# DavidHan008/SLAM-1

Hardware: AMD Instinct MI355X
Metric: frames/sec tracking+local-BA @1280x720 (higher is better)
Workload: dtype u8+f32+f64

## Files before the change

### include/slam355.h

```cpp
#ifndef SLAM355_H
#define SLAM355_H

#include <stddef.h>
#include <stdint.h>

#ifdef __cplusplus
extern "C" {
#endif

#define SLAM355_ABI_VERSION 1

#define SLAM_OK 0
#define SLAM_ERR_ARG (-1)
#define SLAM_ERR_HIP (-2)
#define SLAM_ERR_WORKSPACE (-3)
#define SLAM_ERR_COMM (-4)

int slam_abi_version(void);
const char* slam_last_error(void);
int slam_device_count(void);

int slam_hamming_knn2(const uint8_t* d_q, const int32_t* d_nq, int q_cap,
                      const uint8_t* d_t, const int32_t* d_nt, int t_cap,
                      int batch, int32_t* d_idx2, int32_t* d_dist2,
// ... 19 lines not shown

int slam_fundamental_lmeds(const double* d_m1, const double* d_m2, const int32_t* d_count,
                           int cap, int batch, uint64_t seed, int item0, int n_hyp,
                           uint8_t* d_mask, double* d_F, int32_t* d_ninliers, void* stream);
int slam_fundamental_lmeds_ws(const double* d_m1, const double* d_m2, const int32_t* d_count,
                              int cap, int batch, uint64_t seed, int item0, int n_hyp,
                              uint8_t* d_mask, double* d_F, int32_t* d_ninliers, double* d_ws,
                              long long ws_len, void* stream);
long long slam_fundamental_workspace_len(int batch, int n_hyp);

int slam_filter_pairs(const int32_t* d_pairs, const int32_t* d_count, const uint8_t* d_mask,
                      int cap, int batch, int32_t* d_out, int32_t* d_out_count, void* stream);

int slam_triangulate(const double* d_ptl, const double* d_ptr, const int32_t* d_count, int cap,
                     int batch, const double* d_Pl, const double* d_Pr, int proj_stride,
                     double* d_X, void* stream);

int slam_pnp_ransac(const double* d_Q, const double* d_q, const int32_t* d_count, int cap,
                    int batch, const double* d_K, uint64_t seed, int item0, int n_hyp,
                    double reproj_thresh, int hyp_iters, int refine_iters, double* d_rvec,
                    double* d_tvec, int32_t* d_ninliers, uint8_t* d_mask, double* d_ws,
                    long long ws_len, void* stream);
long long slam_pnp_workspace_len(int batch, int n_hyp);

int slam_pose_chain(const double* d_rvec, const double* d_tvec, const int32_t* d_ninliers,
                    int batch, double* d_state, double* d_poses, void* stream);

int slam_vo_estimate_pose(const double* d_q1, const double* d_q2, const double* d_Q1,
                          const double* d_Q2, const int32_t* d_count, int cap, int batch,
                          const double* d_P, uint64_t seed, int item0, int max_iter,
                          int lm_iters, int early_stop, double* d_pose, int32_t* d_best,
                          int32_t* d_ntried, double* d_err, void* d_ws, size_t ws_bytes,
                          void* stream);
int slam_vo_pose_workspace_bytes(int batch, int max_iter, size_t* bytes);

int slam_vo_residuals(const double* d_dof, const double* d_q1, const double* d_q2,
                      const double* d_Q1, const double* d_Q2, const int32_t* d_count, int cap,
                      int batch, const double* d_P, double* d_res, void* stream);

int slam_rel_to_abs(const double* d_rel, const int32_t* d_count, int cap, int batch,
                    const double* d_poses, double* d_abs, void* stream);

int slam_map_workspace_bytes(int max_queries, int map_cap, size_t* bytes);
int slam_map_associate(double* d_map, int32_t* d_M, int map_cap, int M_bound,
                       const double* d_abs, const double* d_rel, const double* d_pts2d,
                       const int32_t* d_n, int N, double threshold, int frame_index,
// ... 218 lines not shown
```

### slam-1_amd/csrc/epnp.hpp

```cpp
#pragma once

#include <hip/hip_runtime.h>
#include <cmath>

namespace slam_epnp {

constexpr int EPNP_MAXN = 8;
constexpr int kEpnpWs = 4 * EPNP_MAXN + 48 + 60;

template <int n>
__device__ __forceinline__ void ep_jacobi(double* A, double* V) {
  #pragma unroll
  for (int i = 0; i < n; ++i)
    #pragma unroll
    for (int j = 0; j < n; ++j) V[i * n + j] = i == j ? 1.0 : 0.0;
  #pragma unroll 1
  for (int sweep = 0; sweep < 40; ++sweep) {
    double off = 0.0, dia = 0.0;
    #pragma unroll
    for (int i = 0; i < n; ++i) {
      dia += A[i * n + i] * A[i * n + i];
      #pragma unroll
      for (int j = i + 1; j < n; ++j) off += A[i * n + j] * A[i * n + j];
    }
    if (!(off > 1e-30 * dia)) break;
    constexpr int kUnroll = n <= 4 ? 4 : 1;
// ... 218 lines not shown
  } else if (R[0] > R[4] && R[0] > R[8]) {
    const double s = 2.0 * sqrt(1.0 + R[0] - R[4] - R[8]);
    q0 = (R[7] - R[5]) / s; q1 = 0.25 * s; q2 = (R[1] + R[3]) / s; q3 = (R[2] + R[6]) / s;
  } else if (R[4] > R[8]) {
    const double s = 2.0 * sqrt(1.0 + R[4] - R[0] - R[8]);
    q0 = (R[2] - R[6]) / s; q1 = (R[1] + R[3]) / s; q2 = 0.25 * s; q3 = (R[5] + R[7]) / s;
  } else {
    const double s = 2.0 * sqrt(1.0 + R[8] - R[0] - R[4]);
    q0 = (R[3] - R[1]) / s; q1 = (R[2] + R[6]) / s; q2 = (R[5] + R[7]) / s; q3 = 0.25 * s;
  }
  if (q0 < 0.0) {
    q0 = -q0; q1 = -q1; q2 = -q2; q3 = -q3;
  }
  const double vn = sqrt(q1 * q1 + q2 * q2 + q3 * q3);
  const double th = 2.0 * atan2(vn, q0);
  const double k = vn > 0.0 ? th / vn : 2.0;
  r[0] = q1 * k; r[1] = q2 * k; r[2] = q3 * k;
}

constexpr int kJld = 13;
struct EpGroup {
  double A[144], V[144];
  double alph[4 * EPNP_MAXN];
  double v[4][12];
  double L[60], rho[6];
  double cw[4][3];
  double res[3][8];
  double offdia[2];
  double B[2][12 * kJld];
  double cs[12];
  double part[24];
  double pad[27];
  int flag;
};
static_assert(sizeof(EpGroup) % 256 == 128, "EpGroup stride must be 128 mod 256 bytes");

template <int n>
__device__ __forceinline__ int ep_bary(const double* pw, EpGroup& G) {
  double cw[4][3] = {{0, 0, 0}};
  for (int i = 0; i < n; ++i)
    for (int d = 0; d < 3; ++d) cw[0][d] += pw[3 * i + d];
  for (int d = 0; d < 3; ++d) cw[0][d] /= n;
  double A3[9] = {0, 0, 0, 0, 0, 0, 0, 0, 0}, V3[9];
  for (int i = 0; i < n; ++i)
    for (int a = 0; a < 3; ++a)
      for (int b = 0; b < 3; ++b) A3[3 * a + b] += (pw[3 * i + a] - cw[0][a]) * (pw[3 * i + b] - cw[0][b]);
  ep_jacobi<3>(A3, V3);
  int ord[3] = {0, 1, 2};
  for (int i = 0; i < 3; ++i)
    for (int j = i + 1; j < 3; ++j)
      if (A3[4 * ord[j]] > A3[4 * ord[i]]) {
        const int tmp = ord[i]; ord[i] = ord[j]; ord[j] = tmp;
      }
  for (int k = 0; k < 3; ++k) {
    const double sc = sqrt(fmax(A3[4 * ord[k]], 0.0) / n);
    for (int d = 0; d < 3; ++d) cw[k + 1][d] = cw[0][d] + sc * V3[3 * d + ord[k]];
  }
  for (int k = 0; k < 4; ++k)
// ... 186 lines not shown
    ep_jacobi_round<0>(G, k, kr, act, cur, vr);
    ep_jacobi_round<1>(G, k, kr, act, cur ^ 1, vr);
    ep_jacobi_round<2>(G, k, kr, act, cur, vr);
    ep_jacobi_round<3>(G, k, kr, act, cur ^ 1, vr);
    ep_jacobi_round<4>(G, k, kr, act, cur, vr);
    ep_jacobi_round<5>(G, k, kr, act, cur ^ 1, vr);
    ep_jacobi_round<6>(G, k, kr, act, cur, vr);
    ep_jacobi_round<7>(G, k, kr, act, cur ^ 1, vr);
    ep_jacobi_round<8>(G, k, kr, act, cur, vr);
    ep_jacobi_round<9>(G, k, kr, act, cur ^ 1, vr);
    ep_jacobi_round<10>(G, k, kr, act, cur, vr);
    cur ^= 1;
  }
  if (own) {
#pragma unroll
    for (int j = 0; j < n; ++j) {
      G.A[k * n + j] = G.B[cur][k * ld + j];
      G.V[k * n + j] = vr[j];
    }
  }
  __syncthreads();
}

__device__ __forceinline__ void ep_lrho(EpGroup& G) {
  int o12[12];
  for (int i = 0; i < 12; ++i) o12[i] = i;
  for (int i = 0; i < 4; ++i)
    for (int j = i + 1; j < 12; ++j)
      if (G.A[13 * o12[j]] < G.A[13 * o12[i]]) {
        const int tmp = o12[i]; o12[i] = o12[j]; o12[j] = tmp;
      }
  for (int k = 0; k < 4; ++k)
    for (int r = 0; r < 12; ++r) G.v[k][r] = G.V[12 * r + o12[k]];
  const int pa[6] = {0, 0, 0, 1, 1, 2}, pb[6] = {1, 2, 3, 2, 3, 3};
  for (int j = 0; j < 6; ++j) {
    double dv[4][3];
    for (int k = 0; k < 4; ++k)
      for (int d = 0; d < 3; ++d) dv[k][d] = G.v[k][3 * pa[j] + d] - G.v[k][3 * pb[j] + d];
#define EP_DOT(a, b) (dv[a][0] * dv[b][0] + dv[a][1] * dv[b][1] + dv[a][2] * dv[b][2])
    G.L[10 * j + 0] = EP_DOT(0, 0);
    G.L[10 * j + 1] = 2.0 * EP_DOT(0, 1);
    G.L[10 * j + 2] = EP_DOT(1, 1);
    G.L[10 * j + 3] = 2.0 * EP_DOT(0, 2);
    G.L[10 * j + 4] = 2.0 * EP_DOT(1, 2);
    G.L[10 * j + 5] = EP_DOT(2, 2);
    G.L[10 * j + 6] = 2.0 * EP_DOT(0, 3);
    G.L[10 * j + 7] = 2.0 * EP_DOT(1, 3);
    G.L[10 * j + 8] = 2.0 * EP_DOT(2, 3);
    G.L[10 * j + 9] = EP_DOT(3, 3);
#undef EP_DOT
    double s = 0.0;
    for (int d = 0; d < 3; ++d) {
      const double e = G.cw[pa[j]][d] - G.cw[pb[j]][d];
      s += e * e;
    }
    G.rho[j] = s;
  }
}

template <int n>
__device__ __forceinline__ void ep_approx(int approx, const double* pw, const double* uv, double fx,
                                          double fy, double cx, double cy, EpGroup& G) {
  double* res = G.res[approx];
  res[7] = 0.0;
  const int k = approx == 0 ? 4 : approx == 1 ? 3 : 5;
  double As[30], xb[5], rho[6];
#pragma unroll
  for (int j = 0; j < 6; ++j) rho[j] = G.rho[j];
#pragma unroll
  for (int j = 0; j < 6; ++j)
#pragma unroll
    for (int c = 0; c < 5; ++c) {
      const int col = c < 2 ? c : approx == 0 ? (c == 2 ? 3 : 6) : c;
      As[j * 5 + c] = c < k ? G.L[10 * j + col] : 0.0;
    }
  if (!ep_lsq6_live(As, rho, k, xb)) return;
  double be[4] = {0, 0, 0, 0};
  if (approx == 0) {
    if (xb[0] < 0.0) {
      be[0] = sqrt(-xb[0]);
      be[1] = -xb[1] / be[0]; be[2] = -xb[2] / be[0]; be[3] = -xb[3] / be[0];
    } else {
      be[0] = sqrt(xb[0]);
      be[1] = xb[1] / be[0]; be[2] = xb[2] / be[0]; be[3] = xb[3] / be[0];
    }
// ... 21 lines not shown
      Ag[4 * j + 3] = l[6] * be[0] + l[7] * be[1] + l[8] * be[2] + 2.0 * l[9] * be[3];
      bg[j] = rho[j] - (l[0] * be[0] * be[0] + l[1] * be[0] * be[1] + l[2] * be[1] * be[1] +
                        l[3] * be[0] * be[2] + l[4] * be[1] * be[2] + l[5] * be[2] * be[2] +
                        l[6] * be[0] * be[3] + l[7] * be[1] * be[3] + l[8] * be[2] * be[3] +
                        l[9] * be[3] * be[3]);
    }
    if (!ep_lsq6<4>(Ag, bg, dx)) break;
    for (int c = 0; c < 4; ++c) be[c] += dx[c];
  }
  double ccs[4][3];
  for (int j = 0; j < 4; ++j)
    for (int d = 0; d < 3; ++d)
      ccs[j][d] = be[0] * G.v[0][3 * j + d] + be[1] * G.v[1][3 * j + d] + be[2] * G.v[2][3 * j + d] +
                  be[3] * G.v[3][3 * j + d];
  double R[9], t[3];
  res[0] = ep_pose<n>(ccs, G.alph, pw, uv, fx, fy, cx, cy, R, t);
  double r[3];
  ep_rvec(R, r);
  res[1] = r[0]; res[2] = r[1]; res[3] = r[2];
  res[4] = t[0]; res[5] = t[1]; res[6] = t[2];
  res[7] = 1.0;
}

__device__ __forceinline__ int ep_choose(const EpGroup& G, double p[6]) {
  double best_err = INFINITY;
  int ok = 0;
  for (int a = 0; a < 3; ++a) {
    if (G.res[a][7] == 0.0) continue;
    if (G.res[a][0] < best_err) {
      best_err = G.res[a][0];
      for (int i = 0; i < 6; ++i) p[i] = G.res[a][1 + i];
      ok = 1;
    }
  }
  for (int i = 0; i < 6; ++i) ok &= isfinite(p[i]) ? 1 : 0;
  return ok;
}

}
```

### slam-1_amd/csrc/geometry.hip

```cpp
#include "common.hpp"
#include "epnp.hpp"
#include "dlt.hpp"

#include <climits>

#include <cmath>

namespace {

constexpr int kBS = 256;

__global__ __launch_bounds__(kBS) void k_gather(const float* __restrict__ kpq, int kq_cap,
                                                const float* __restrict__ kpt, int kt_cap,
                                                const uint8_t* __restrict__ dq_in,
                                                const uint8_t* __restrict__ dt_in,
                                                const int2* __restrict__ pairs,
                                                const int32_t* __restrict__ count, int p_cap,
                                                double* __restrict__ ptq, double* __restrict__ ptt,
                                                uint8_t* __restrict__ dq, uint8_t* __restrict__ dt) {
  const int b = blockIdx.y;
  const int n = min(max(count[b], 0), p_cap);
  const int k = blockIdx.x * kBS + threadIdx.x;
  if (k >= n) return;
  const size_t o = (size_t)b * p_cap + k;
// ... 269 lines not shown
__device__ __forceinline__ void allsum_halve(double (&v)[32], int lane) {
  constexpr int half = OFF / 2;
  const bool hi = (lane & OFF) != 0;
#pragma unroll
  for (int k = 0; k < half; ++k) {
    const double send = hi ? v[k] : v[k + half];
    const double keep = hi ? v[k + half] : v[k];
    v[k] = keep + __shfl_xor(send, OFF, 64);
  }
}
__device__ __forceinline__ void wave_allsum32(double (&v)[32]) {
  const int lane = threadIdx.x & 63;
  allsum_halve<32>(v, lane);
  allsum_halve<16>(v, lane);
  allsum_halve<8>(v, lane);
  allsum_halve<4>(v, lane);
  allsum_halve<2>(v, lane);
  const double tot = v[0] + __shfl_xor(v[0], 1, 64);
#pragma unroll
  for (int j = 0; j < 32; ++j) v[j] = readlane_d(tot, 2 * j);
}

constexpr int kHypGroups = 4;
#ifdef SLAM_PNPH_TRACE
__device__ unsigned long long g_pnph[8];
#define PNPH_T(i) do { if (threadIdx.x == 0 && blockIdx.x == 3 && blockIdx.y == 5) g_pnph[i] = __builtin_amdgcn_s_memtime(); } while (0)
#else
#define PNPH_T(i) (void)0
#endif
__device__ void pnp_sample(uint64_t seed, int item, int h, int L, const double* Q, const double* q,
                           double* pw, double* uv, int* sidx) {
  uint64_t s = seed ^ ((uint64_t)item * 0xD1B54A32D192ED03ull) ^
               ((uint64_t)h * 0x8CB92BA72F3D8DD7ull);
  int idx[kMinSample];
  for (int kk = 0; kk < kMinSample; ++kk) {
    int v;
    bool dup;
    do {
      v = (int)((splitmix64(s) >> 32) % (uint64_t)L);
      dup = false;
      for (int j = 0; j < kk; ++j) dup |= idx[j] == v;
    } while (dup);
    idx[kk] = v;
    sidx[kk] = v;
    for (int d = 0; d < 3; ++d) pw[3 * kk + d] = Q[3 * v + d];
    for (int d = 0; d < 2; ++d) uv[2 * kk + d] = q[2 * v + d];
  }
}

__global__ __launch_bounds__(64) void k_pnp_hyp(const double* __restrict__ Qall,
                                                const double* __restrict__ qall,
                                                const int32_t* __restrict__ count, int cap,
                                                const double* __restrict__ Kp, uint64_t seed,
                                                int item0, int n_hyp, double* __restrict__ ws) {
#ifdef SLAM_PNP_PRIO
  __builtin_amdgcn_s_setprio(SLAM_PNP_PRIO);
#endif
  __shared__ slam_epnp::EpGroup grp[kHypGroups];
  __shared__ double spw[kHypGroups][3 * kMinSample], suv[kHypGroups][2 * kMinSample];
  __shared__ int sidx[kHypGroups][kMinSample];
  const int b = blockIdx.x, t = threadIdx.x;
  const int g = t >> 4, k = t & 15;
  const int h = blockIdx.y * kHypGroups + g;
  const int L = min(max(count[b], 0), cap);
  if (L < kMinSample) return;
  const bool live = h < n_hyp;
  const double* Q = Qall + (size_t)b * cap * 3;
  const double* q = qall + (size_t)b * cap * 2;
  const Cam K{Kp[0], Kp[4], Kp[2], Kp[5]};
  slam_epnp::EpGroup& G = grp[g];
  PNPH_T(0);
  if (k == 0 && live) {
    pnp_sample(seed, item0 + b, h, L, Q, q, spw[g], suv[g], sidx[g]);
    G.flag = slam_epnp::ep_bary<kMinSample>(spw[g], G);
  }
  __syncthreads();
  PNPH_T(1);
  bool ok = live && G.flag != 0;
  if (ok && k < 12) slam_epnp::ep_mtm_row<kMinSample>(k, suv[g], K.fx, K.fy, K.cx, K.cy, G);
  __syncthreads();
  PNPH_T(2);
  slam_epnp::ep_jacobi12_group(G, k, ok);
  PNPH_T(3);
#ifdef SLAM_PNPH_TRACE
  if (threadIdx.x == 0 && blockIdx.x == 3 && blockIdx.y == 5) g_pnph[7] = (unsigned long long)G.offdia[1];
#endif
  if (ok && k == 0) slam_epnp::ep_lrho(G);
  __syncthreads();
  PNPH_T(4);
  if (ok && k < 3) slam_epnp::ep_approx<kMinSample>(k, spw[g], suv[g], K.fx, K.fy, K.cx, K.cy, G);
  __syncthreads();
  PNPH_T(5);
  if (k == 0 && live) {
    double p[6] = {0, 0, 0, 0, 0, 0};
    if (!(ok && slam_epnp::ep_choose(G, p)))
      for (int i = 0; i < 6; ++i) p[i] = 0.0;
    double* o = ws + ((size_t)b * n_hyp + h) * 6;
    for (int i = 0; i < 6; ++i) o[i] = p[i];
  }
  PNPH_T(6);
}

__global__ __launch_bounds__(64) void k_pnp_hyp_lm(const double* __restrict__ Qall,
                                                   const double* __restrict__ qall,
                                                   const int32_t* __restrict__ count, int cap,
                                                   const double* __restrict__ Kp, uint64_t seed,
                                                   int item0, int n_hyp, int hyp_iters,
                                                   double* __restrict__ ws) {
#ifdef SLAM_PNP_PRIO
  __builtin_amdgcn_s_setprio(SLAM_PNP_PRIO);
#endif
  __shared__ double spw[kHypGroups][3 * kMinSample], suv[kHypGroups][2 * kMinSample];
  __shared__ int sidx[kHypGroups][kMinSample];
  __shared__ double lmt[kHypGroups * kLmGroup], lms[kHypGroups][28 + kMinSample];
  __shared__ double p0[kHypGroups][6];
  const int b = blockIdx.x, t = threadIdx.x;
  const int g = t >> 4, k = t & 15;
  const int h = blockIdx.y * kHypGroups + g;
  const int L = min(max(count[b], 0), cap);
  if (L < kMinSample) return;
  const bool live = h < n_hyp;
  const double* Q = Qall + (size_t)b * cap * 3;
  const double* q = qall + (size_t)b * cap * 2;
// ... 610 lines not shown
      d_Q1, d_q2, d_q1);
  SLAM_LAUNCHED("k_gather_temporal");
  return SLAM_OK;
}

extern "C" int slam_triangulate(const double* d_ptl, const double* d_ptr, const int32_t* d_count,
                                int cap, int batch, const double* d_Pl, const double* d_Pr,
                                int proj_stride, double* d_X, void* stream) {
  SLAM_REQUIRE(batch >= 0 && cap >= 0, "slam_triangulate: bad shape");
  SLAM_REQUIRE(proj_stride == 0 || proj_stride == 12, "slam_triangulate: proj_stride 0 or 12");
  if (batch == 0 || cap == 0) return SLAM_OK;
  SLAM_REQUIRE(d_ptl && d_ptr && d_count && d_Pl && d_Pr && d_X, "slam_triangulate: null pointer");
  dim3 grid((cap + kBS - 1) / kBS, batch);
  k_triangulate<<<grid, kBS, 0, slam::as_stream(stream)>>>(d_ptl, d_ptr, d_count, cap, d_Pl, d_Pr,
                                                           proj_stride, d_X);
  SLAM_LAUNCHED("k_triangulate");
  return SLAM_OK;
}

extern "C" long long slam_pnp_workspace_len(int batch, int n_hyp) {
  return (long long)batch * n_hyp * 6;
}

extern "C" int slam_pnp_ransac(const double* d_Q, const double* d_q, const int32_t* d_count,
                               int cap, int batch, const double* d_K, uint64_t seed, int item0,
                               int n_hyp, double reproj_thresh, int hyp_iters, int refine_iters,
                               double* d_rvec, double* d_tvec, int32_t* d_ninliers,
                               uint8_t* d_mask, double* d_ws, long long ws_len, void* stream) {
  SLAM_REQUIRE(batch >= 0 && cap >= 0, "slam_pnp_ransac: bad shape");
  SLAM_REQUIRE(n_hyp >= 1 && n_hyp <= kMaxHyp, "slam_pnp_ransac: n_hyp in [1, %d]", kMaxHyp);
  SLAM_REQUIRE(hyp_iters >= 0 && refine_iters >= 0 && reproj_thresh > 0,
               "slam_pnp_ransac: bad iteration/threshold arguments");
  if (batch == 0) return SLAM_OK;
  SLAM_REQUIRE(d_Q && d_q && d_count && d_K && d_rvec && d_tvec && d_ninliers && d_mask && d_ws,
               "slam_pnp_ransac: null pointer");
  if (ws_len < slam_pnp_workspace_len(batch, n_hyp)) {
    slam::set_error("slam_pnp_ransac: workspace %lld < %lld doubles", ws_len,
                    slam_pnp_workspace_len(batch, n_hyp));
    return SLAM_ERR_WORKSPACE;
  }
  hipStream_t s = slam::as_stream(stream);
  const dim3 hgrid(batch, (n_hyp + kHypGroups - 1) / kHypGroups);
  k_pnp_hyp<<<hgrid, 64, 0, s>>>(d_Q, d_q, d_count, cap, d_K, seed, item0, n_hyp, d_ws);
  SLAM_LAUNCHED("k_pnp_hyp");
  k_pnp_hyp_lm<<<hgrid, 64, 0, s>>>(d_Q, d_q, d_count, cap, d_K, seed, item0, n_hyp, hyp_iters,
                                    d_ws);
  SLAM_LAUNCHED("k_pnp_hyp_lm");
  k_pnp<<<batch, kPnPWG, 0, s>>>(d_Q, d_q, d_count, cap, d_K, seed, item0, n_hyp, reproj_thresh,
                                 hyp_iters, refine_iters, d_rvec, d_tvec, d_ninliers, d_mask,
                                 d_ws);
  SLAM_LAUNCHED("k_pnp");
  return SLAM_OK;
}

extern "C" int slam_vo_pose_workspace_bytes(int batch, int max_iter, size_t* bytes) {
  SLAM_REQUIRE(batch >= 0 && max_iter >= 1 && bytes, "slam_vo_pose_workspace_bytes: bad args");
  *bytes = (size_t)batch * max_iter * 7 * sizeof(double) + 256;
  return SLAM_OK;
}

extern "C" int slam_vo_estimate_pose(const double* d_q1, const double* d_q2, const double* d_Q1,
                                     const double* d_Q2, const int32_t* d_count, int cap,
                                     int batch, const double* d_P, uint64_t seed, int item0,
                                     int max_iter, int lm_iters, int early_stop, double* d_pose,
                                     int32_t* d_best, int32_t* d_ntried, double* d_err,
                                     void* d_ws, size_t ws_bytes, void* stream) {
  SLAM_REQUIRE(batch >= 0 && cap >= 0, "slam_vo_estimate_pose: bad shape");
  SLAM_REQUIRE(max_iter >= 1 && max_iter <= kVoWG, "slam_vo_estimate_pose: max_iter in [1, %d]",
               kVoWG);
  SLAM_REQUIRE(lm_iters >= 0 && early_stop >= 1, "slam_vo_estimate_pose: bad lm_iters/early_stop");
  if (batch == 0) return SLAM_OK;
  SLAM_REQUIRE(d_q1 && d_q2 && d_Q1 && d_Q2 && d_count && d_P && d_pose && d_best && d_ntried &&
                   d_err,
               "slam_vo_estimate_pose: null pointer");
  SLAM_REQUIRE(d_ws != nullptr, "slam_vo_estimate_pose: null workspace");
// ... 29 lines not shown
               "slam_vo_residuals: null pointer");
  dim3 grid((4 * cap + kBS - 1) / kBS, batch);
  k_vo_residuals<<<grid, kBS, 0, slam::as_stream(stream)>>>(d_dof, d_q1, d_q2, d_Q1, d_Q2,
                                                           d_count, cap, d_P, d_res);
  SLAM_LAUNCHED("k_vo_residuals");
  return SLAM_OK;
}

extern "C" int slam_pose_chain(const double* d_rvec, const double* d_tvec,
                               const int32_t* d_ninliers, int batch, double* d_state,
                               double* d_poses, void* stream) {
  SLAM_REQUIRE(batch >= 0, "slam_pose_chain: batch < 0");
  if (batch == 0) return SLAM_OK;
  SLAM_REQUIRE(d_rvec && d_tvec && d_ninliers && d_state && d_poses, "slam_pose_chain: null pointer");
  k_pose_chain<<<1, 64, 0, slam::as_stream(stream)>>>(d_rvec, d_tvec, d_ninliers, batch, d_state,
                                                     d_poses);
  SLAM_LAUNCHED("k_pose_chain");
  return SLAM_OK;
}

#ifdef SLAM_PNPH_TRACE
extern "C" int slam_pnph_trace(unsigned long long* out) {
  SLAM_HIP(hipDeviceSynchronize());
  SLAM_HIP(hipMemcpyFromSymbol(out, HIP_SYMBOL(g_pnph), 8 * sizeof(unsigned long long)));
  return SLAM_OK;
}
#endif
```

### slam-1_amd/slam355/_lib.py

```python
from __future__ import annotations

import ctypes
import os

_HERE = os.path.dirname(os.path.abspath(__file__))
LIB_PATH = os.environ.get("SLAM355_LIB") or os.path.join(_HERE, "libslam355.so")

c_int = ctypes.c_int
c_double = ctypes.c_double
c_size_t = ctypes.c_size_t
c_p = ctypes.c_void_p
c_uint64 = ctypes.c_uint64
c_longlong = ctypes.c_longlong

c_i32 = ctypes.c_int32


class BAProblemStruct(ctypes.Structure):
    _fields_ = [
        ("n_cams", c_i32), ("n_pts", c_i32), ("n_obs", c_i32), ("n_grps", c_i32),
        ("n_blocks", c_i32), ("n_cslots", c_i32), ("n_bslots", c_i32), ("lin_mode", c_i32),
        ("n_sgrps", c_i32), ("tl_mode", c_i32),
        ("cams", c_p * 2), ("pts", c_p * 2), ("camrec", c_p * 2),
        ("obs_cam", c_p), ("obs_pt", c_p), ("obs_q", c_p), ("pt_ptr", c_p), ("grp_ptr", c_p),
# ... 24 lines not shown
        ("n_cslots", c_i32), ("n_bslots", c_i32), ("n_blocks", c_i32), ("chunks_per_wg", c_i32),
        ("off", ctypes.c_longlong * len(PLAN_TABLES)), ("len", ctypes.c_longlong * len(PLAN_TABLES)),
        ("total", ctypes.c_longlong),
    ]

SIGNATURES = {
    "slam_abi_version": [],
    "slam_last_error": [],
    "slam_device_count": [],
    "slam_hamming_knn2": [c_p, c_p, c_int, c_p, c_p, c_int, c_int, c_p, c_p, c_p, c_p],
    "slam_compact_matches": [c_p, c_p, c_p, c_int, c_int, c_p, c_double, c_p, c_p, c_p],
    "slam_orb_workspace_bytes": [c_int, c_int, c_int, c_int, c_int, c_int, c_int,
                                 ctypes.POINTER(c_size_t)],
    "slam_orb_tiles": [c_p, c_int, c_int, c_int, c_int, c_int, c_int, c_int, c_int, c_p,
                       c_size_t, c_p, c_p, c_p, c_p, c_int, c_p],
    "slam_gather_matches": [c_p, c_int, c_p, c_int, c_p, c_p, c_p, c_p, c_int, c_int, c_p, c_p,
                            c_p, c_p, c_p],
    "slam_gather_temporal": [c_p, c_p, c_int, c_p, c_int, c_p, c_p, c_int, c_int, c_p, c_p, c_p,
                             c_p],
    "slam_triangulate": [c_p, c_p, c_p, c_int, c_int, c_p, c_p, c_int, c_p, c_p],
    "slam_pnp_ransac": [c_p, c_p, c_p, c_int, c_int, c_p, c_uint64, c_int, c_int, c_double, c_int,
                        c_int, c_p, c_p, c_p, c_p, c_p, c_longlong, c_p],
    "slam_pnp_workspace_len": [c_int, c_int],
    "slam_pose_chain": [c_p, c_p, c_p, c_int, c_p, c_p, c_p],
    "slam_vo_estimate_pose": [c_p, c_p, c_p, c_p, c_p, c_int, c_int, c_p, c_uint64, c_int, c_int,
                              c_int, c_int, c_p, c_p, c_p, c_p, c_p, c_size_t, c_p],
    "slam_vo_pose_workspace_bytes": [c_int, c_int, ctypes.POINTER(c_size_t)],
    "slam_vo_residuals": [c_p, c_p, c_p, c_p, c_p, c_p, c_int, c_int, c_p, c_p, c_p],
    "slam_map_workspace_bytes": [c_int, c_int, ctypes.POINTER(c_size_t)],
    "slam_rel_to_abs": [c_p, c_p, c_int, c_int, c_p, c_p, c_p],
    "slam_map_windows": [c_p, c_p, c_int, c_int, c_int, c_p, c_p, c_p, c_p, c_int, c_double, c_p,
                         c_p, c_size_t, c_p],
    "slam_map_associate": [c_p, c_p, c_int, c_int, c_p, c_p, c_p, c_p, c_int, c_double, c_int,
                           c_p, c_p, c_size_t, c_p],
    "slam_fundamental_lmeds": [c_p, c_p, c_p, c_int, c_int, c_uint64, c_int, c_int, c_p, c_p, c_p,
                               c_p],
    "slam_fundamental_lmeds_ws": [c_p, c_p, c_p, c_int, c_int, c_uint64, c_int, c_int, c_p, c_p,
                                  c_p, c_p, c_longlong, c_p],
    "slam_fundamental_workspace_len": [c_int, c_int],
    "slam_filter_pairs": [c_p, c_p, c_p, c_int, c_int, c_p, c_p, c_p],
    "slam_ba_residual": [c_p, c_p, c_p, c_p, c_p, c_int, c_p, c_p],
    "slam_ba_jacobian": [c_p, c_p, c_p, c_p, c_p, c_int, c_p, c_p, c_p],
    "slam_ba_red_slots": [c_int],
    "slam_ba_problem_size": [],
    "slam_ba_sys_len": [c_int, c_int],
    "slam_ba_chol_len": [c_int, c_p],
# ... 31 lines not shown
    "slam_sgbm": [c_p, c_p, c_int, c_int, c_int, c_int, c_int, c_int, c_int, c_int, c_int, c_p,
                  c_size_t, c_p, c_p, c_p],
    "slam_vo_right_qs_3d": [c_p, c_p, c_p, c_int, c_int, c_p, ctypes.c_longlong,
                            ctypes.c_longlong, c_int, c_int, ctypes.c_float, ctypes.c_float, c_p,
                            c_p, c_p, c_p, c_p, c_p, c_p, c_p, c_p, c_p, c_p, c_p, c_p, c_p],
    "slam_triangulate_f32": [c_p, c_p, c_p, c_int, c_int, c_p, c_p, c_p, c_p],
    "slam_pose_chain_trf": [c_p, c_int, c_int, c_int, c_int, c_double, c_double, c_double, c_int,
                            c_p, c_p],
    "slam_comm_unique_id": [c_p],
    "slam_comm_init": [c_int, c_int, c_p, ctypes.POINTER(c_p)],
    "slam_comm_destroy": [c_p],
    "slam_comm_allreduce_f64": [c_p, c_p, ctypes.c_longlong, c_p],
    "slam_ba_step_distributed": [_PROB, c_p, c_p],
    "slam_ba_plan_bound": [c_int, c_int, c_int, c_int],
    "slam_ba_plan_mfma": [c_int, c_int, c_int, c_p, c_p, c_p, c_int, c_int, c_p, c_longlong,
                          ctypes.POINTER(PlanInfo)],
    "slam_ba_stage_windows": [c_int, c_int, c_int, c_p, c_p, c_p, c_int, c_p, c_p, c_double,
                              c_double, c_p, c_longlong, c_p, c_longlong, c_p, c_p, c_p, c_p, c_p],
}
_RESTYPE = {"slam_last_error": ctypes.c_char_p, "slam_ba_sys_len": ctypes.c_longlong,
            "slam_ba_plan_bound": ctypes.c_longlong,
            "slam_ba_chol_len": ctypes.c_longlong, "slam_ba_cov_workspace_len": ctypes.c_longlong,
            "slam_pnp_workspace_len": ctypes.c_longlong,
            "slam_fundamental_workspace_len": ctypes.c_longlong,
            "slam_pose_chain_workspace_len": ctypes.c_longlong}


class SlamError(RuntimeError):
    """A libslam355 call returned a non-zero status."""


def _load():
    if not os.path.exists(LIB_PATH):
        raise ImportError(
            f"libslam355.so not found at {LIB_PATH}: build it with "
            "`make -C slam-1_amd` (or __graft_entry__.build()). slam355 has no CPU fallback."
        )
    import torch

    lib = ctypes.CDLL(LIB_PATH)
    for name, argtypes in SIGNATURES.items():
        fn = getattr(lib, name)
        fn.argtypes = argtypes
        fn.restype = _RESTYPE.get(name, c_int)
    return lib

# ... 13 lines not shown
```

### slam-1_amd/slam355/geometry.py

```python
from __future__ import annotations

import ctypes

import numpy as np
import torch

from . import _lib
from .device import ptr, require_gpu, stream_ptr

PNP_DEFAULTS = dict(n_hyp=100, reproj_thresh=8.0, hyp_iters=10, refine_iters=20)


def gather_matches(kpq, kpt, pairs, count, desq=None, dest=None, out=None, stream=None):
    B, p_cap, _ = pairs.shape
    dev = pairs.device
    if out is None:
        ptq = torch.zeros((B, p_cap, 2), dtype=torch.float64, device=dev)
        ptt = torch.zeros((B, p_cap, 2), dtype=torch.float64, device=dev)
        dq = dt = None
        if desq is not None:
            dq = torch.zeros((B, p_cap, 32), dtype=torch.uint8, device=dev)
            dt = torch.zeros((B, p_cap, 32), dtype=torch.uint8, device=dev)
    else:
        ptq, ptt, dq, dt = out
# ... 46 lines not shown
        o = torch.empty_like(pairs)
        oc = torch.empty((B,), dtype=torch.int32, device=pairs.device)
    else:
        o, oc = out
    _lib.call("slam_filter_pairs", ptr(pairs), ptr(count), ptr(mask), cap, B, ptr(o), ptr(oc),
              stream_ptr(stream))
    return o, oc


def triangulate(ptl, ptr_, count, P_l, P_r, out=None, stream=None):
    B, cap, _ = ptl.shape
    Pl = P_l if isinstance(P_l, torch.Tensor) else torch.as_tensor(np.asarray(P_l, np.float64),
                                                                   device=ptl.device)
    Pr = P_r if isinstance(P_r, torch.Tensor) else torch.as_tensor(np.asarray(P_r, np.float64),
                                                                   device=ptl.device)
    Pl, Pr = Pl.contiguous(), Pr.contiguous()
    stride = 12 if Pl.dim() == 3 else 0
    X = out if out is not None else torch.zeros((B, cap, 3), dtype=torch.float64, device=ptl.device)
    _lib.call("slam_triangulate", ptr(ptl), ptr(ptr_), ptr(count), cap, B, ptr(Pl), ptr(Pr), stride,
              ptr(X), stream_ptr(stream))
    return X


def pnp_ransac(Q, q, count, K, seed=0, item0=0, out=None, stream=None, ws=None, **kw):
    prm = dict(PNP_DEFAULTS, **kw)
    B, cap, _ = Q.shape
    dev = Q.device
    Kt = K if isinstance(K, torch.Tensor) else torch.as_tensor(np.asarray(K, np.float64), device=dev)
    if out is None:
        rvec = torch.zeros((B, 3), dtype=torch.float64, device=dev)
        tvec = torch.zeros((B, 3), dtype=torch.float64, device=dev)
        ninl = torch.zeros((B,), dtype=torch.int32, device=dev)
        mask = torch.zeros((B, max(cap, 1)), dtype=torch.uint8, device=dev)
    else:
        rvec, tvec, ninl, mask = out
    if ws is None:
        ws = pnp_workspace(B, prm["n_hyp"], dev)
        if stream is not None and stream != torch.cuda.current_stream(dev):
            ws.record_stream(stream)
    _lib.call("slam_pnp_ransac", ptr(Q), ptr(q), ptr(count), cap, B, ptr(Kt.contiguous()),
              int(seed) & ((1 << 64) - 1), int(item0), prm["n_hyp"], float(prm["reproj_thresh"]),
              prm["hyp_iters"], prm["refine_iters"], ptr(rvec), ptr(tvec), ptr(ninl), ptr(mask),
              ptr(ws), ws.numel(), stream_ptr(stream))
    return rvec, tvec, ninl, mask


def pnp_workspace(B, n_hyp=PNP_DEFAULTS["n_hyp"], dev="cuda"):
    n = int(_lib.lib.slam_pnp_workspace_len(B, n_hyp))
    return torch.empty(max(n, 1), dtype=torch.float64, device=dev)


VO_DEFAULTS = dict(max_iter=100, lm_iters=20, early_stop=5)


def vo_estimate_pose(q1, q2, Q1, Q2, count, P, seed=0, item0=0, out=None, stream=None, **kw):
    prm = dict(VO_DEFAULTS, **kw)
    B, cap, _ = Q1.shape
    dev = Q1.device
    Pt = P if isinstance(P, torch.Tensor) else torch.as_tensor(np.asarray(P, np.float64), device=dev)
    if out is None:
        pose = torch.zeros((B, 6), dtype=torch.float64, device=dev)
        best = torch.zeros((B,), dtype=torch.int32, device=dev)
        ntried = torch.zeros((B,), dtype=torch.int32, device=dev)
        err = torch.zeros((B,), dtype=torch.float64, device=dev)
    else:
        pose, best, ntried, err = out
    nb = ctypes.c_size_t(0)
    _lib.call("slam_vo_pose_workspace_bytes", B, prm["max_iter"], ctypes.byref(nb))
    ws = torch.empty(nb.value, dtype=torch.uint8, device=dev)
    _lib.call("slam_vo_estimate_pose", ptr(q1), ptr(q2), ptr(Q1), ptr(Q2), ptr(count), cap, B,
              ptr(Pt.contiguous()), int(seed) & ((1 << 64) - 1), int(item0), prm["max_iter"],
# ... 15 lines not shown
```

### slam-1_amd/slam355/pipeline.py

```python
from __future__ import annotations

import time

import numpy as np
import torch

from . import _lib, geometry, matcher, orb
from .device import ptr, require_gpu, stream_ptr


class Tracker:

    def __init__(self, B, H, W, P_l, P_r, max_kp_per_tile=56, seed=0, max_distance=500.0,
                 stream=None, orb_stream=None):
        self.dev = require_gpu()
        self.B, self.H, self.W = B, H, W
        self.max_kp = max_kp_per_tile
        self.seed = seed
        self.max_distance = float(max_distance)
        self.stream = stream
        self.P_l = np.asarray(P_l, np.float64)
        self.P_r = np.asarray(P_r, np.float64)
        self.K = self.P_l[:3, :3].copy()
        d = self.dev
# ... 21 lines not shown
        self.f_mask = torch.zeros((B, cap), **u8)
        self.f_F = torch.zeros((B, 9), **f64)
        self.f_ninl = torch.zeros((B,), **i32)
        self.f_pairs = torch.zeros((B, cap, 2), **i32)
        self.f_cnt = torch.zeros((B,), **i32)
        self.f_ptl = torch.zeros((B, cap, 2), **f64)
        self.f_ptr = torch.zeros((B, cap, 2), **f64)
        self.f_dl = torch.zeros((B, cap, 32), **u8)
        self.f_dr = torch.zeros((B, cap, 32), **u8)
        self.X = torch.zeros((B, cap, 3), **f64)
        self.t_idx2 = torch.full((B, cap, 2), -1, **i32)
        self.t_dist2 = torch.full((B, cap, 2), -1, **i32)
        self.t_good = torch.zeros((B, cap), **u8)
        self.t_pairs = torch.zeros((B, cap, 2), **i32)
        self.t_cnt = torch.zeros((B,), **i32)
        self.Q1 = torch.zeros((B, cap, 3), **f64)
        self.q2 = torch.zeros((B, cap, 2), **f64)
        self.q1 = torch.zeros((B, cap, 2), **f64)
        self.rvec = torch.zeros((B, 3), **f64)
        self.tvec = torch.zeros((B, 3), **f64)
        self.p_ninl = torch.zeros((B,), **i32)
        self.p_mask = torch.zeros((B, cap), **u8)
        self.p_ws = geometry.pnp_workspace(B, dev=d)
        self.f_ws = geometry.fundamental_workspace(B, dev=d)
        self.imgs = torch.zeros((2 * B + 1, H, W), **u8)
        self.chain_state = torch.zeros((32,), **f64)
        self._chain_eye = torch.from_numpy(np.concatenate([np.eye(4), np.eye(4)]).ravel()).to(d)
        self.reset_chain()
        self.poses = torch.zeros((B, 4, 4), **f64)
        self.orb_min = torch.full((1,), 1 << 30, **i32)
        self.orb_event = torch.cuda.Event()
        self.host_times = None

    def _ht(self, site, t0):
        t1 = time.perf_counter()
        if self.host_times is not None:
            self.host_times.setdefault(site, []).append(t1 - t0)
        return t1

    def track(self, frame0: int, imgs: torch.Tensor | None = None, marks=None, chain=True):
        B, st = self.B, self.stream
        im = self.imgs if imgs is None else imgs

        def mark(name):
            if marks is not None:
                ev = torch.cuda.Event(enable_timing=True)
# ... 44 lines not shown
        h0 = self._ht("stereo_launch", h0)
        geometry.fundamental_lmeds(self.s_ptl, self.s_ptr, self.s_cnt, seed=self.seed,
                                   item0=frame0, out=(self.f_mask, self.f_F, self.f_ninl),
                                   stream=st, ws=self.f_ws)
        mark("f_lmeds")
        geometry.filter_pairs(self.s_pairs, self.s_cnt, self.f_mask,
                              out=(self.f_pairs, self.f_cnt), stream=st)
        geometry.gather_matches(kpL, kpR, self.f_pairs, self.f_cnt, dL, dR,
                                out=(self.f_ptl, self.f_ptr, self.f_dl, self.f_dr), stream=st)
        geometry.triangulate(self.f_ptl, self.f_ptr, self.f_cnt, self.tPl, self.tPr, out=self.X,
                             stream=st)
        matcher.knn2_batch(self.f_dl, self.f_cnt, dL1, nL1,
                           out=(self.t_idx2, self.t_dist2, self.t_good), stream=st)
        matcher.compact_matches(self.t_idx2, self.t_good, self.f_cnt, gate_xyz=self.X,
                                gate=self.max_distance, out=(self.t_pairs, self.t_cnt), stream=st)
        geometry.gather_temporal(self.X, self.f_ptl, kpL1, self.t_pairs, self.t_cnt,
                                 out=(self.Q1, self.q2, self.q1), stream=st)
        if ost is not None:
            self.slot_free[slot].record(main)
        mark("triangulate_temporal")
        h0 = self._ht("flmeds_tri_temporal_launch", h0)
        geometry.pnp_ransac(self.Q1, self.q2, self.t_cnt, self.tK, seed=self.seed, item0=frame0,
                            out=(self.rvec, self.tvec, self.p_ninl, self.p_mask), stream=st,
                            ws=self.p_ws)
        mark("pnp")
        h0 = self._ht("pnp_launch", h0)
        if chain:
            _lib.call("slam_pose_chain", ptr(self.rvec), ptr(self.tvec), ptr(self.p_ninl), B,
                      ptr(self.chain_state), ptr(self.poses), stream_ptr(st))
            mark("pose_chain")
            self._ht("pose_chain_launch", h0)
        return self.rvec, self.tvec, self.p_ninl

    def reset_chain(self, pose0=None, T0=None):
        with torch.cuda.stream(self.stream if self.stream is not None
                               else torch.cuda.current_stream()):
            if pose0 is None and T0 is None:
                src = self._chain_eye
            else:
                st = np.concatenate([np.eye(4) if pose0 is None else np.asarray(pose0, float),
                                     np.eye(4) if T0 is None else np.asarray(T0, float)]).ravel()
                src = torch.from_numpy(st).to(self.chain_state.device)
            self.chain_state.copy_(src, non_blocking=True)

    def check(self):
        cur = torch.cuda.current_stream()
        streams = [x for x in (self.stream, self.orb_stream) if x is not None]
# ... 159 lines not shown
```

Baseline: 23030.

## Split EPnP hypothesis kernel into eigen and beta stages via global scratch

Splits the PnP hypothesis kernel into two kernels. The first runs the Jacobi eigen-decomposition with 4 hypotheses per block and writes a compact per-hypothesis record (sample points, alphas, control points, the four smallest eigenvectors) to a global scratch buffer. The second packs 16 hypotheses per block into a smaller shared-memory EpBeta struct and does the L/rho, approximations and choice steps. This shrinks the shared footprint of the eigen stage and packs more hypotheses per block in the serial beta stage, at the cost of an extra kernel launch and a scratch round-trip through global memory. The pipeline preallocates the scratch buffer; the legacy entry point allocates it per call with hipMallocAsync.

```diff
diff --git a/include/slam355.h b/include/slam355.h
--- a/include/slam355.h
+++ b/include/slam355.h
@@ -65,6 +65,12 @@
                     double* d_tvec, int32_t* d_ninliers, uint8_t* d_mask, double* d_ws,
                     long long ws_len, void* stream);
 long long slam_pnp_workspace_len(int batch, int n_hyp);
+int slam_pnp_ransac_ws(const double* d_Q, const double* d_q, const int32_t* d_count, int cap,
+                       int batch, const double* d_K, uint64_t seed, int item0, int n_hyp,
+                       double reproj_thresh, int hyp_iters, int refine_iters, double* d_rvec,
+                       double* d_tvec, int32_t* d_ninliers, uint8_t* d_mask, double* d_ws,
+                       long long ws_len, double* d_scratch, long long scratch_len, void* stream);
+long long slam_pnp_scratch_len(int batch, int n_hyp);
 
 int slam_pose_chain(const double* d_rvec, const double* d_tvec, const int32_t* d_ninliers,
                     int batch, double* d_state, double* d_poses, void* stream);
diff --git a/slam-1_amd/csrc/epnp.hpp b/slam-1_amd/csrc/epnp.hpp
--- a/slam-1_amd/csrc/epnp.hpp
+++ b/slam-1_amd/csrc/epnp.hpp
@@ -2,6 +2,7 @@
 
 #include <hip/hip_runtime.h>
 #include <cmath>
+#include <cstddef>
 
 namespace slam_epnp {
 
@@ -266,18 +267,29 @@
 struct EpGroup {
   double A[144], V[144];
   double alph[4 * EPNP_MAXN];
-  double v[4][12];
-  double L[60], rho[6];
   double cw[4][3];
-  double res[3][8];
   double offdia[2];
   double B[2][12 * kJld];
   double cs[12];
   double part[24];
-  double pad[27];
+  double pad[3];
+  int o12[4];
   int flag;
 };
 static_assert(sizeof(EpGroup) % 256 == 128, "EpGroup stride must be 128 mod 256 bytes");
+
+struct EpBeta {
+  double flag;
+  double pw[3 * 5], uv[2 * 5];
+  double alph[4 * 5];
+  double cw[4][3];
+  double v[4][12];
+  double L[60], rho[6];
+  double res[3][8];
+};
+constexpr int kEpRec = 1 + 15 + 10 + 20 + 12 + 48;
+static_assert(offsetof(EpBeta, L) == kEpRec * sizeof(double), "EpBeta starts with the record");
+static_assert(sizeof(EpBeta) % 64 == 32, "EpBeta stride must be 4 mod 8 doubles");
 
 template <int n>
 __device__ __forceinline__ int ep_bary(const double* pw, EpGroup& G) {
@@ -510,7 +522,7 @@
   __syncthreads();
 }
 
-__device__ __forceinline__ void ep_lrho(EpGroup& G) {
+__device__ __forceinline__ void ep_order(EpGroup& G) {
   int o12[12];
   for (int i = 0; i < 12; ++i) o12[i] = i;
   for (int i = 0; i < 4; ++i)
@@ -518,8 +530,10 @@
       if (G.A[13 * o12[j]] < G.A[13 * o12[i]]) {
         const int tmp = o12[i]; o12[i] = o12[j]; o12[j] = tmp;
       }
-  for (int k = 0; k < 4; ++k)
-    for (int r = 0; r < 12; ++r) G.v[k][r] = G.V[12 * r + o12[k]];
+  for (int k = 0; k < 4; ++k) G.o12[k] = o12[k];
+}
+
+__device__ __forceinline__ void ep_lrho(EpBeta& G) {
   const int pa[6] = {0, 0, 0, 1, 1, 2}, pb[6] = {1, 2, 3, 2, 3, 3};
   for (int j = 0; j < 6; ++j) {
     double dv[4][3];
@@ -548,7 +562,7 @@
 
 template <int n>
 __device__ __forceinline__ void ep_approx(int approx, const double* pw, const double* uv, double fx,
-                                          double fy, double cx, double cy, EpGroup& G) {
+                                          double fy, double cx, double cy, EpBeta& G) {
   double* res = G.res[approx];
   res[7] = 0.0;
   const int k = approx == 0 ? 4 : approx == 1 ? 3 : 5;
@@ -616,7 +630,7 @@
   res[7] = 1.0;
 }
 
-__device__ __forceinline__ int ep_choose(const EpGroup& G, double p[6]) {
+__device__ __forceinline__ int ep_choose(const EpBeta& G, double p[6]) {
   double best_err = INFINITY;
   int ok = 0;
   for (int a = 0; a < 3; ++a) {
diff --git a/slam-1_amd/csrc/geometry.hip b/slam-1_amd/csrc/geometry.hip
--- a/slam-1_amd/csrc/geometry.hip
+++ b/slam-1_amd/csrc/geometry.hip
@@ -315,8 +315,10 @@
 }
 
 constexpr int kHypGroups = 4;
+constexpr int kBetaGroups = 16;
+constexpr int kEpRec = slam_epnp::kEpRec;
 #ifdef SLAM_PNPH_TRACE
-__device__ unsigned long long g_pnph[8];
+__device__ unsigned long long g_pnph[16];
 #define PNPH_T(i) do { if (threadIdx.x == 0 && blockIdx.x == 3 && blockIdx.y == 5) g_pnph[i] = __builtin_amdgcn_s_memtime(); } while (0)
 #else
 #define PNPH_T(i) (void)0
@@ -341,11 +343,12 @@
   }
 }
 
-__global__ __launch_bounds__(64) void k_pnp_hyp(const double* __restrict__ Qall,
-                                                const double* __restrict__ qall,
-                                                const int32_t* __restrict__ count, int cap,
-                                                const double* __restrict__ Kp, uint64_t seed,
-                                                int item0, int n_hyp, double* __restrict__ ws) {
+__global__ __launch_bounds__(64) void k_pnp_hyp_eig(const double* __restrict__ Qall,
+                                                    const double* __restrict__ qall,
+                                                    const int32_t* __restrict__ count, int cap,
+                                                    const double* __restrict__ Kp, uint64_t seed,
+                                                    int item0, int n_hyp,
+                                                    double* __restrict__ scr) {
 #ifdef SLAM_PNP_PRIO
   __builtin_amdgcn_s_setprio(SLAM_PNP_PRIO);
 #endif
@@ -378,12 +381,58 @@
 #ifdef SLAM_PNPH_TRACE
   if (threadIdx.x == 0 && blockIdx.x == 3 && blockIdx.y == 5) g_pnph[7] = (unsigned long long)G.offdia[1];
 #endif
+  if (ok && k == 0) slam_epnp::ep_order(G);
+  __syncthreads();
+  if (live) {
+    double* rec = scr + ((size_t)b * n_hyp + h) * kEpRec;
+    if (k == 0) rec[0] = ok ? 1.0 : 0.0;
+    if (ok) {
+      if (k < 3 * kMinSample) rec[1 + k] = spw[g][k];
+      if (k < 2 * kMinSample) rec[16 + k] = suv[g][k];
+      for (int i = k; i < 4 * kMinSample; i += 16) rec[26 + i] = G.alph[i];
+      if (k < 12) {
+        rec[46 + k] = G.cw[k / 3][k % 3];
+        for (int kk = 0; kk < 4; ++kk) rec[58 + 12 * kk + k] = G.V[12 * k + G.o12[kk]];
+      }
+    }
+  }
+  PNPH_T(4);
+}
+
+__global__ __launch_bounds__(64) void k_pnp_hyp_beta(const int32_t* __restrict__ count, int cap,
+                                                     const double* __restrict__ Kp, int n_hyp,
+                                                     const double* __restrict__ scr,
+                                                     double* __restrict__ ws) {
+#ifdef SLAM_PNP_PRIO
+  __builtin_amdgcn_s_setprio(SLAM_PNP_PRIO);
+#endif
+  __shared__ slam_epnp::EpBeta grp[kBetaGroups];
+  const int b = blockIdx.x, t = threadIdx.x;
+  const int g = t >> 2, k = t & 3;
+  const int h0 = blockIdx.y * kBetaGroups, h = h0 + g;
+  const int L = min(max(count[b], 0), cap);
+  if (L < kMinSample) return;
+  const bool live = h < n_hyp;
+  const Cam K{Kp[0], Kp[4], Kp[2], Kp[5]};
+  slam_epnp::EpBeta& G = grp[g];
+  PNPH_T(8);
+  {
+    const double* src = scr + ((size_t)b * n_hyp + h0) * kEpRec;
+    const int nrec = min(kBetaGroups, n_hyp - h0) * kEpRec;
+    for (int i = t; i < nrec; i += 64) {
+      const int gi = i / kEpRec;
+      reinterpret_cast<double*>(&grp[gi])[i - gi * kEpRec] = src[i];
+    }
+  }
+  __syncthreads();
+  PNPH_T(9);
+  const bool ok = live && G.flag != 0.0;
   if (ok && k == 0) slam_epnp::ep_lrho(G);
   __syncthreads();
-  PNPH_T(4);
-  if (ok && k < 3) slam_epnp::ep_approx<kMinSample>(k, spw[g], suv[g], K.fx, K.fy, K.cx, K.cy, G);
+  PNPH_T(10);
+  if (ok && k < 3) slam_epnp::ep_approx<kMinSample>(k, G.pw, G.uv, K.fx, K.fy, K.cx, K.cy, G);
   __syncthreads();
-  PNPH_T(5);
+  PNPH_T(11);
   if (k == 0 && live) {
     double p[6] = {0, 0, 0, 0, 0, 0};
     if (!(ok && slam_epnp::ep_choose(G, p)))
@@ -391,7 +440,7 @@
     double* o = ws + ((size_t)b * n_hyp + h) * 6;
     for (int i = 0; i < 6; ++i) o[i] = p[i];
   }
-  PNPH_T(6);
+  PNPH_T(12);
 }
 
 __global__ __launch_bounds__(64) void k_pnp_hyp_lm(const double* __restrict__ Qall,
@@ -1048,11 +1097,11 @@
   return (long long)batch * n_hyp * 6;
 }
 
-extern "C" int slam_pnp_ransac(const double* d_Q, const double* d_q, const int32_t* d_count,
-                               int cap, int batch, const double* d_K, uint64_t seed, int item0,
-                               int n_hyp, double reproj_thresh, int hyp_iters, int refine_iters,
-                               double* d_rvec, double* d_tvec, int32_t* d_ninliers,
-                               uint8_t* d_mask, double* d_ws, long long ws_len, void* stream) {
+static int pnp_check_args(const double* d_Q, const double* d_q, const int32_t* d_count, int cap,
+                          int batch, const double* d_K, int n_hyp, double reproj_thresh,
+                          int hyp_iters, int refine_iters, const double* d_rvec,
+                          const double* d_tvec, const int32_t* d_ninliers, const uint8_t* d_mask,
+                          const double* d_ws, long long ws_len) {
   SLAM_REQUIRE(batch >= 0 && cap >= 0, "slam_pnp_ransac: bad shape");
   SLAM_REQUIRE(n_hyp >= 1 && n_hyp <= kMaxHyp, "slam_pnp_ransac: n_hyp in [1, %d]", kMaxHyp);
   SLAM_REQUIRE(hyp_iters >= 0 && refine_iters >= 0 && reproj_thresh > 0,
@@ -1065,11 +1114,37 @@
                     slam_pnp_workspace_len(batch, n_hyp));
     return SLAM_ERR_WORKSPACE;
   }
+  return SLAM_OK;
+}
+
+extern "C" long long slam_pnp_scratch_len(int batch, int n_hyp) {
+  return (long long)(batch > 0 ? batch : 0) * (n_hyp > 0 ? n_hyp : 0) * kEpRec;
+}
+
+extern "C" int slam_pnp_ransac_ws(const double* d_Q, const double* d_q, const int32_t* d_count,
+                                  int cap, int batch, const double* d_K, uint64_t seed, int item0,
+                                  int n_hyp, double reproj_thresh, int hyp_iters, int refine_iters,
+                                  double* d_rvec, double* d_tvec, int32_t* d_ninliers,
+                                  uint8_t* d_mask, double* d_ws, long long ws_len,
+                                  double* d_scratch, long long scratch_len, void* stream) {
+  if (int rc = pnp_check_args(d_Q, d_q, d_count, cap, batch, d_K, n_hyp, reproj_thresh, hyp_iters,
+                              refine_iters, d_rvec, d_tvec, d_ninliers, d_mask, d_ws, ws_len))
+    return rc;
+  if (batch == 0) return SLAM_OK;
+  SLAM_REQUIRE(d_scratch != nullptr, "slam_pnp_ransac: null scratch");
+  if (scratch_len < slam_pnp_scratch_len(batch, n_hyp)) {
+    slam::set_error("slam_pnp_ransac: scratch %lld < %lld doubles", scratch_len,
+                    slam_pnp_scratch_len(batch, n_hyp));
+    return SLAM_ERR_WORKSPACE;
+  }
   hipStream_t s = slam::as_stream(stream);
-  const dim3 hgrid(batch, (n_hyp + kHypGroups - 1) / kHypGroups);
-  k_pnp_hyp<<<hgrid, 64, 0, s>>>(d_Q, d_q, d_count, cap, d_K, seed, item0, n_hyp, d_ws);
-  SLAM_LAUNCHED("k_pnp_hyp");
-  k_pnp_hyp_lm<<<hgrid, 64, 0, s>>>(d_Q, d_q, d_count, cap, d_K, seed, item0, n_hyp, hyp_iters,
+  const dim3 egrid(batch, (n_hyp + kHypGroups - 1) / kHypGroups);
+  k_pnp_hyp_eig<<<egrid, 64, 0, s>>>(d_Q, d_q, d_count, cap, d_K, seed, item0, n_hyp, d_scratch);
+  SLAM_LAUNCHED("k_pnp_hyp_eig");
+  const dim3 bgrid(batch, (n_hyp + kBetaGroups - 1) / kBetaGroups);
+  k_pnp_hyp_beta<<<bgrid, 64, 0, s>>>(d_count, cap, d_K, n_hyp, d_scratch, d_ws);
+  SLAM_LAUNCHED("k_pnp_hyp_beta");
+  k_pnp_hyp_lm<<<egrid, 64, 0, s>>>(d_Q, d_q, d_count, cap, d_K, seed, item0, n_hyp, hyp_iters,
                                     d_ws);
   SLAM_LAUNCHED("k_pnp_hyp_lm");
   k_pnp<<<batch, kPnPWG, 0, s>>>(d_Q, d_q, d_count, cap, d_K, seed, item0, n_hyp, reproj_thresh,
@@ -1077,6 +1152,26 @@
                                  d_ws);
   SLAM_LAUNCHED("k_pnp");
   return SLAM_OK;
+}
+
+extern "C" int slam_pnp_ransac(const double* d_Q, const double* d_q, const int32_t* d_count,
+                               int cap, int batch, const double* d_K, uint64_t seed, int item0,
+                               int n_hyp, double reproj_thresh, int hyp_iters, int refine_iters,
+                               double* d_rvec, double* d_tvec, int32_t* d_ninliers,
+                               uint8_t* d_mask, double* d_ws, long long ws_len, void* stream) {
+  if (int rc = pnp_check_args(d_Q, d_q, d_count, cap, batch, d_K, n_hyp, reproj_thresh, hyp_iters,
+                              refine_iters, d_rvec, d_tvec, d_ninliers, d_mask, d_ws, ws_len))
+    return rc;
+  if (batch == 0) return SLAM_OK;
+  hipStream_t s = slam::as_stream(stream);
+  const long long n = slam_pnp_scratch_len(batch, n_hyp);
+  double* scr = nullptr;
+  SLAM_HIP(hipMallocAsync(reinterpret_cast<void**>(&scr), (size_t)n * sizeof(double), s));
+  const int rc = slam_pnp_ransac_ws(d_Q, d_q, d_count, cap, batch, d_K, seed, item0, n_hyp,
+                                    reproj_thresh, hyp_iters, refine_iters, d_rvec, d_tvec,
+                                    d_ninliers, d_mask, d_ws, ws_len, scr, n, s);
+  SLAM_HIP(hipFreeAsync(scr, s));
+  return rc;
 }
 
 extern "C" int slam_vo_pose_workspace_bytes(int batch, int max_iter, size_t* bytes) {
@@ -1152,7 +1247,7 @@
 #ifdef SLAM_PNPH_TRACE
 extern "C" int slam_pnph_trace(unsigned long long* out) {
   SLAM_HIP(hipDeviceSynchronize());
-  SLAM_HIP(hipMemcpyFromSymbol(out, HIP_SYMBOL(g_pnph), 8 * sizeof(unsigned long long)));
+  SLAM_HIP(hipMemcpyFromSymbol(out, HIP_SYMBOL(g_pnph), 16 * sizeof(unsigned long long)));
   return SLAM_OK;
 }
 #endif
diff --git a/slam-1_amd/slam355/_lib.py b/slam-1_amd/slam355/_lib.py
--- a/slam-1_amd/slam355/_lib.py
+++ b/slam-1_amd/slam355/_lib.py
@@ -70,6 +70,9 @@
     "slam_pnp_ransac": [c_p, c_p, c_p, c_int, c_int, c_p, c_uint64, c_int, c_int, c_double, c_int,
                         c_int, c_p, c_p, c_p, c_p, c_p, c_longlong, c_p],
     "slam_pnp_workspace_len": [c_int, c_int],
+    "slam_pnp_ransac_ws": [c_p, c_p, c_p, c_int, c_int, c_p, c_uint64, c_int, c_int, c_double,
+                           c_int, c_int, c_p, c_p, c_p, c_p, c_p, c_longlong, c_p, c_longlong, c_p],
+    "slam_pnp_scratch_len": [c_int, c_int],
     "slam_pose_chain": [c_p, c_p, c_p, c_int, c_p, c_p, c_p],
     "slam_vo_estimate_pose": [c_p, c_p, c_p, c_p, c_p, c_int, c_int, c_p, c_uint64, c_int, c_int,
                               c_int, c_int, c_p, c_p, c_p, c_p, c_p, c_size_t, c_p],
@@ -147,6 +150,7 @@
             "slam_ba_plan_bound": ctypes.c_longlong,
             "slam_ba_chol_len": ctypes.c_longlong, "slam_ba_cov_workspace_len": ctypes.c_longlong,
             "slam_pnp_workspace_len": ctypes.c_longlong,
+            "slam_pnp_scratch_len": ctypes.c_longlong,
             "slam_fundamental_workspace_len": ctypes.c_longlong,
             "slam_pose_chain_workspace_len": ctypes.c_longlong}
 
diff --git a/slam-1_amd/slam355/geometry.py b/slam-1_amd/slam355/geometry.py
--- a/slam-1_amd/slam355/geometry.py
+++ b/slam-1_amd/slam355/geometry.py
@@ -92,7 +92,8 @@
     return X
 
 
-def pnp_ransac(Q, q, count, K, seed=0, item0=0, out=None, stream=None, ws=None, **kw):
+def pnp_ransac(Q, q, count, K, seed=0, item0=0, out=None, stream=None, ws=None, scratch=None,
+               **kw):
     prm = dict(PNP_DEFAULTS, **kw)
     B, cap, _ = Q.shape
     dev = Q.device
@@ -108,15 +109,24 @@
         ws = pnp_workspace(B, prm["n_hyp"], dev)
         if stream is not None and stream != torch.cuda.current_stream(dev):
             ws.record_stream(stream)
-    _lib.call("slam_pnp_ransac", ptr(Q), ptr(q), ptr(count), cap, B, ptr(Kt.contiguous()),
-              int(seed) & ((1 << 64) - 1), int(item0), prm["n_hyp"], float(prm["reproj_thresh"]),
-              prm["hyp_iters"], prm["refine_iters"], ptr(rvec), ptr(tvec), ptr(ninl), ptr(mask),
-              ptr(ws), ws.numel(), stream_ptr(stream))
+    args = (ptr(Q), ptr(q), ptr(count), cap, B, ptr(Kt.contiguous()),
+            int(seed) & ((1 << 64) - 1), int(item0), prm["n_hyp"], float(prm["reproj_thresh"]),
+            prm["hyp_iters"], prm["refine_iters"], ptr(rvec), ptr(tvec), ptr(ninl), ptr(mask),
+            ptr(ws), ws.numel())
+    if scratch is None:
+        _lib.call("slam_pnp_ransac", *args, stream_ptr(stream))
+    else:
+        _lib.call("slam_pnp_ransac_ws", *args, ptr(scratch), scratch.numel(), stream_ptr(stream))
     return rvec, tvec, ninl, mask
 
 
 def pnp_workspace(B, n_hyp=PNP_DEFAULTS["n_hyp"], dev="cuda"):
     n = int(_lib.lib.slam_pnp_workspace_len(B, n_hyp))
+    return torch.empty(max(n, 1), dtype=torch.float64, device=dev)
+
+
+def pnp_scratch(B, n_hyp=PNP_DEFAULTS["n_hyp"], dev="cuda"):
+    n = int(_lib.lib.slam_pnp_scratch_len(B, n_hyp))
     return torch.empty(max(n, 1), dtype=torch.float64, device=dev)
 
 
diff --git a/slam-1_amd/slam355/pipeline.py b/slam-1_amd/slam355/pipeline.py
--- a/slam-1_amd/slam355/pipeline.py
+++ b/slam-1_amd/slam355/pipeline.py
@@ -67,6 +67,7 @@
         self.p_ninl = torch.zeros((B,), **i32)
         self.p_mask = torch.zeros((B, cap), **u8)
         self.p_ws = geometry.pnp_workspace(B, dev=d)
+        self.p_scr = geometry.pnp_scratch(B, dev=d)
         self.f_ws = geometry.fundamental_workspace(B, dev=d)
         self.imgs = torch.zeros((2 * B + 1, H, W), **u8)
         self.chain_state = torch.zeros((32,), **f64)
@@ -157,7 +158,7 @@
         h0 = self._ht("flmeds_tri_temporal_launch", h0)
         geometry.pnp_ransac(self.Q1, self.q2, self.t_cnt, self.tK, seed=self.seed, item0=frame0,
                             out=(self.rvec, self.tvec, self.p_ninl, self.p_mask), stream=st,
-                            ws=self.p_ws)
+                            ws=self.p_ws, scratch=self.p_scr)
         mark("pnp")
         h0 = self._ht("pnp_launch", h0)
         if chain:
```

New measurement: 23600, median of 6. 1.02x the previous value.
